# robflynnyh/dynamic-asr-eval

Measured on AMD Instinct MI355X. Metric: audio-sec/s dynamic-eval (fwd+1 adapt step), higher is better.
Workload: dtype f32; 1 GPU; run_dynamic_eval_full: 1 h Earnings-22-shape recording per step (360000 frames, seq_len 16384, overlap 14336, offline, MADGRAD lr 9e-05, 6 freq masks <=34), SCConformerXL 6x768 V+1=4096 seeded weights; windows_per_recording=169, chains_per_gpu=2, lockstep_group=4, hip_graphs=True, pcie_inclusive=False

## Files before the change

dynamic-asr-eval_amd/_lib.py:

```python
import ctypes
import os

_HERE = os.path.dirname(os.path.abspath(__file__))
LIB_PATH = os.environ.get("DYN_LIB_PATH") or os.path.join(_HERE, "libdyneval_hip.so")
_lib = None


class DynError(RuntimeError):
    pass


class GemmDesc(ctypes.Structure):
    _fields_ = [
        ("trans_a", ctypes.c_int32), ("trans_b", ctypes.c_int32),
        ("M", ctypes.c_int64), ("N", ctypes.c_int64), ("K", ctypes.c_int64),
        ("alpha", ctypes.c_float), ("beta", ctypes.c_float),
        ("A", ctypes.c_void_p), ("lda", ctypes.c_int64), ("sa1", ctypes.c_int64), ("sa2", ctypes.c_int64),
        ("B", ctypes.c_void_p), ("ldb", ctypes.c_int64), ("sb1", ctypes.c_int64), ("sb2", ctypes.c_int64),
        ("C", ctypes.c_void_p), ("ldc", ctypes.c_int64), ("sc1", ctypes.c_int64), ("sc2", ctypes.c_int64),
        ("bias", ctypes.c_void_p),
        ("nb1", ctypes.c_int64), ("nb2", ctypes.c_int64),
        ("split_k", ctypes.c_int32),
        ("workspace", ctypes.c_void_p), ("workspace_bytes", ctypes.c_int64),
        ("tile_m", ctypes.c_int32), ("tile_n", ctypes.c_int32), ("tail_slices", ctypes.c_int32), ("reserved_", ctypes.c_int32),
        ("C_in", ctypes.c_void_p),
        ("epilogue", ctypes.c_int32), ("reserved2_", ctypes.c_int32),
        ("aux", ctypes.c_void_p),
        ("a_colsum", ctypes.c_void_p),
        ("a_colsum_beta", ctypes.c_float), ("reserved3_", ctypes.c_float),
        ("counters", ctypes.c_void_p), ("n_counters", ctypes.c_int64),
        ("bias_s1", ctypes.c_int64), ("bias_s2", ctypes.c_int64),
    ]


class DecoderDesc(ctypes.Structure):
    _fields_ = [
        ("d_model", ctypes.c_int32), ("heads", ctypes.c_int32), ("d_ff", ctypes.c_int32), ("vocab", ctypes.c_int32),
        ("layers", ctypes.c_int32), ("n_enc", ctypes.c_int32), ("max_positions", ctypes.c_int32), ("reserved_", ctypes.c_int32),
        ("eps", ctypes.c_float), ("reserved2_", ctypes.c_float),
        ("embed", ctypes.c_void_p), ("pos_table", ctypes.c_void_p), ("norm_out_w", ctypes.c_void_p), ("norm_out_b", ctypes.c_void_p),
        ("head_w", ctypes.c_void_p), ("head_b", ctypes.c_void_p),
        ("layer_ptrs", ctypes.POINTER(ctypes.c_void_p)),
        ("tokens", ctypes.c_void_p), ("logits", ctypes.c_void_p), ("scratch", ctypes.c_void_p), ("scratch_floats", ctypes.c_int64),
    ]


class DecoderBatchDesc(ctypes.Structure):
    _fields_ = [
        ("base", DecoderDesc), ("rows", ctypes.c_int32), ("eos_id", ctypes.c_int32),
        ("token_stride", ctypes.c_int64), ("cache_stride", ctypes.c_int64), ("finished", ctypes.c_void_p),
    ]


DEC_PTRS_PER_LAYER = 18


def load():
    global _lib
    if _lib is not None:
        return _lib
    if not os.path.exists(LIB_PATH):
        raise DynError(
            f"{LIB_PATH} not found: the HIP extension has not been built "
            "(run `python -c 'import __graft_entry__ as g; g.build()'` or `make -C dynamic-asr-eval_amd/csrc`). "
            "There is no CPU fallback for the product path.")
    import torch
    lib = ctypes.CDLL(LIB_PATH)
    for name, (restype, argtypes) in prototypes().items():
        fn = getattr(lib, name)
        fn.restype = restype
        fn.argtypes = argtypes
    _lib = lib
    return lib


def check(rc, what=""):
    if rc != 0:
# ... 44 lines not shown
```

dynamic-asr-eval_amd/csrc/gemm_f32.hip:

```cpp
#include <algorithm>
#include "common.h"
#include <cstdlib>

typedef float f32x16 __attribute__((ext_vector_type(16)));

namespace {

#ifndef DYN_GEMM_BK
#define DYN_GEMM_BK 32
#endif
constexpr int BK = DYN_GEMM_BK;
constexpr int LDK = BK + 4;
constexpr int KV = BK / 4;
constexpr int RP = 256 / KV;
constexpr int NTHREADS = 256;

struct KParams {
    int64_t M, N, K;
    const float* A; int64_t lda, sa1, sa2;
    const float* B; int64_t ldb, sb1, sb2;
    float* C; int64_t ldc, sc1, sc2;
    int64_t cin_delta;
    const float* bias;
    int64_t bs1, bs2;
// ... 488 lines not shown
__global__ void splitk_reduce_kernel(const KParams p) {
    const int64_t mn = p.M * p.N;
    const int64_t total = mn * p.nbatch;
    for (int64_t idx = (int64_t)blockIdx.x * blockDim.x + threadIdx.x; idx < total;
         idx += (int64_t)gridDim.x * blockDim.x) {
        const int64_t zb = idx / mn, rem = idx % mn;
        const int64_t row = rem / p.N, col = rem % p.N;
        float s = 0.f;
        for (int k = 0; k < p.splits; ++k) s += p.ws[((int64_t)k * p.nbatch + zb) * mn + rem];
        const int64_t z1 = zb / p.nb2, z2 = zb % p.nb2;
        float* C = p.C + z1 * p.sc1 + z2 * p.sc2 + row * p.ldc + col;
        float v = epi_value(p.alpha, s, p.beta, C + p.cin_delta, p.bias ? p.bias[z1 * p.bs1 + z2 * p.bs2 + col] : 0.f);
        if (p.epi == 1) { if (p.aux) C[p.aux - p.C] = v; v = silu_f(v); }
        else if (p.epi == 2) v *= silu_grad_f(C[p.aux - p.C]);
        *C = v;
    }
}

__global__ __launch_bounds__(256) void tail_reduce_kernel(const KParams p, int BM, int BN, int64_t tail_items) {
    const int per_tile = BM * BN / 4;
    const int64_t total = tail_items * per_tile;
    for (int64_t idx = (int64_t)blockIdx.x * blockDim.x + threadIdx.x; idx < total; idx += (int64_t)gridDim.x * blockDim.x) {
        const int64_t ti = idx / per_tile;
        const int e4 = (int)(idx % per_tile);
        const int r = (e4 * 4) / BN, c = (e4 * 4) % BN;
        const float4* W = reinterpret_cast<const float4*>(p.tail_ws + (ti * p.tail_f) * (int64_t)(BM * BN)) + e4;
        float4 s4 = W[0];
        for (int k = 1; k < p.tail_f; ++k) {
            const float4 v = W[(int64_t)k * per_tile];
            s4.x += v.x; s4.y += v.y; s4.z += v.z; s4.w += v.w;
        }
        const int64_t item = p.full_items + ti;
        const int tile = (int)(item % p.tiles_per_batch);
        const int zb = (int)(item / p.tiles_per_batch);
        const int64_t row = (int64_t)(p.n_major ? tile % p.tiles_m : tile / p.tiles_n) * BM + r;
        const int64_t col0 = (int64_t)(p.n_major ? tile / p.tiles_m : tile % p.tiles_n) * BN + c;
        if (row >= p.M) continue;
        const int64_t z1 = zb / p.nb2, z2 = zb % p.nb2;
        float* C = p.C + z1 * p.sc1 + z2 * p.sc2 + row * p.ldc;
        const float v[4] = {s4.x, s4.y, s4.z, s4.w};
#pragma unroll
        for (int j = 0; j < 4; ++j) {
            const int64_t col = col0 + j;
            if (col < p.N) {
                float o = epi_value(p.alpha, v[j], p.beta, C + col + p.cin_delta, p.bias ? p.bias[z1 * p.bs1 + z2 * p.bs2 + col] : 0.f);
                if (p.epi == 1) { if (p.aux) C[col + (p.aux - p.C)] = o; o = silu_f(o); }
                else if (p.epi == 2) o *= silu_grad_f(C[col + (p.aux - p.C)]);
                C[col] = o;
            }
        }
    }
}

struct Plan {
    int bm, bn, splits;
    int64_t kchunk;
    int64_t ws_bytes;
    int64_t full_items;
    int64_t tail_items;
    int tail_f;
    int64_t tail_ws_bytes;
};

double tile_eff(int bm, int bn) { return bm == 256 ? 0.84 : (bm == 128 && bn == 128) ? 0.80 : (bm == 64 && bn == 64) ? 0.62 : 0.72; }
int tile_occ(int bm, int bn) { return bm == 256 ? 1 : (bm == 64 && bn == 64) ? 4 : (bm == 128 && bn == 128) ? 2 : 3; }

bool glds_eligible(const dyn_gemm_desc* d) {
    auto al16 = [](const void* q) { return (((uintptr_t)q) & 15) == 0; };
    const bool vec = al16(d->A) && al16(d->B) && (d->lda % 4 == 0) && (d->ldb % 4 == 0) && (d->sa1 % 4 == 0) && (d->sa2 % 4 == 0) &&
                     (d->sb1 % 4 == 0) && (d->sb2 % 4 == 0);
    static const bool allow_glds = [] { const char* e = getenv("DYN_GEMM_GLDS"); return !e || atoi(e) != 0; }();
    const bool ta = d->trans_a != 0, tb = d->trans_b != 0;
    return allow_glds && vec && d->K % BK == 0 && d->K > 0 && (!ta || d->M % 4 == 0) && (tb || d->N % 4 == 0) && (!ta || d->M >= 4) && (tb || d->N >= 4);
}

bool eval_config(const dyn_gemm_desc* d, int bm, int bn, int s, int f_req, Plan* out, double* cost) {
    const int64_t batch = d->nb1 * d->nb2;
    const int64_t ktiles = dyn::cdiv(d->K > 0 ? d->K : 1, BK);
    if (s < 1) s = 1;
    if (s > ktiles) s = (int)ktiles;
    const int64_t tiles = dyn::cdiv(d->M, bm) * dyn::cdiv(d->N, bn);
    const int64_t slots = (int64_t)tile_occ(bm, bn) * 256;
    const int64_t kchunk = dyn::cdiv(ktiles, s) * BK;
    const int s_eff = (int)dyn::cdiv(d->K > 0 ? d->K : 1, kchunk);
    const int64_t items = tiles * batch * s_eff;
    const int64_t rounds = items / slots, rem = items % slots;
    int f = 1;
    if (s_eff == 1 && rem > 0 && f_req != 1) {
        f = f_req > 1 ? f_req : (int)(slots / rem);
        const int64_t maxf = ktiles / 2 > 0 ? ktiles / 2 : 1;
        if (f > maxf) f = (int)maxf;
        if (f > 16) f = 16;
        if (f < 1) f = 1;
    }
    const double round_t = tile_occ(bm, bn) * 2.0 * bm * bn * (double)kchunk / (614e9 * tile_eff(bm, bn));
    double t = rounds * round_t + (rem > 0 ? round_t / f + 1.0e-6 : 0.0);
    if (s_eff > 1) t += 3e-6 + (double)s_eff * d->M * d->N * batch * 4.0 * 2.0 / 3.0e12;
    if (f > 1) t += 2e-6 + (double)f * rem * bm * bn * 4.0 * 2.0 / 3.0e12;
    *cost = t;
    out->bm = bm; out->bn = bn; out->splits = s_eff; out->kchunk = kchunk;
    out->ws_bytes = s_eff > 1 ? (int64_t)s_eff * batch * tiles * bm * bn * (int64_t)sizeof(float) : 0;
    out->tail_f = f;
    out->tail_items = f > 1 ? rem : 0;
    out->full_items = items - out->tail_items;
    out->tail_ws_bytes = f > 1 ? rem * f * (int64_t)bm * bn * (int64_t)sizeof(float) : 0;
    return true;
}

struct Tuned { int ta, tb; int64_t M, N, K, batch; int bm, bn, split, tail; };
#include "gemm_tuned.inc"

Plan make_plan(const dyn_gemm_desc* d) {
    Plan best;
    double cost;
    if (d->tile_m > 0 && d->tile_n > 0) {
        const bool big = d->tile_m >= 256 && d->tile_n >= 128 && glds_eligible(d);
        eval_config(d, big ? 256 : d->tile_m >= 128 ? 128 : 64, d->tile_n >= 128 ? 128 : 64, d->split_k > 0 ? d->split_k : 1,
                    d->tail_slices > 0 ? d->tail_slices : 1, &best, &cost);
        return best;
    }
    const int64_t batch = d->nb1 * d->nb2;
    if (d->split_k == 0) {
        auto less = [](const Tuned& a, const Tuned& b) {
            if (a.ta != b.ta) return a.ta < b.ta;
            if (a.tb != b.tb) return a.tb < b.tb;
            if (a.M != b.M) return a.M < b.M;
            if (a.N != b.N) return a.N < b.N;
            if (a.K != b.K) return a.K < b.K;
            return a.batch < b.batch;
        };
        static const bool sorted = [&] {
            for (int i = 1; i < kNumTuned; ++i)
                if (!less(kTuned[i - 1], kTuned[i])) return false;
            return true;
        }();
        const Tuned want{d->trans_a != 0, d->trans_b != 0, d->M, d->N, d->K, batch, 0, 0, 0, 0};
        const Tuned* hit = nullptr;
        if (sorted) {
            const Tuned* it = std::lower_bound(kTuned, kTuned + kNumTuned, want, less);
            if (it != kTuned + kNumTuned && !less(want, *it)) hit = it;
        } else {
            for (int i = 0; i < kNumTuned && !hit; ++i)
                if (!less(kTuned[i], want) && !less(want, kTuned[i])) hit = &kTuned[i];
        }
        if (hit) {
            eval_config(d, (hit->bm == 256 && !glds_eligible(d)) ? 128 : hit->bm, hit->bn, hit->split, hit->tail, &best, &cost);
            return best;
        }
    }
    const int cand[4][2] = {{128, 128}, {128, 64}, {64, 128}, {64, 64}};
    int split_opts[9] = {1, 2, 3, 4, 6, 8, 12, 16, 24};
    int n_opts = 9;
    if (d->split_k > 0) { split_opts[0] = d->split_k; n_opts = 1; }
    double best_cost = 1e300;
    for (int c = 0; c < 4; ++c) {
        const int bm = cand[c][0], bn = cand[c][1];
        if ((d->M <= 64 && bm == 128) || (d->N <= 64 && bn == 128)) continue;
        for (int so = 0; so < n_opts; ++so) {
            const int s = split_opts[so];
            if (d->split_k == 0 && s > 1 && (d->K / s < 256)) continue;
            Plan pl;
            eval_config(d, bm, bn, s, d->split_k == 0 ? -1 : 1, &pl, &cost);
            if (cost < best_cost) { best_cost = cost; best = pl; }
        }
    }
    return best;
}

template <bool TA, bool TB, int BM, int BN>
void launch_vec(const KParams& kp, bool vec, dim3 grid, hipStream_t st) {
    static const bool allow_glds = [] { const char* e = getenv("DYN_GEMM_GLDS"); return !e || atoi(e) != 0; }();
    const bool glds = allow_glds && vec && kp.K % BK == 0 && kp.K > 0 && (!TA || kp.M % 4 == 0) && (TB || kp.N % 4 == 0) &&
                      (!TA || kp.M >= 4) && (TB || kp.N >= 4);
    if (glds) hipLaunchKernelGGL((gemm_f32_kernel<TA, TB, BM, BN, true, true>), grid, dim3(NTHREADS), 0, st, kp);
    else if (vec) hipLaunchKernelGGL((gemm_f32_kernel<TA, TB, BM, BN, true, false>), grid, dim3(NTHREADS), 0, st, kp);
    else hipLaunchKernelGGL((gemm_f32_kernel<TA, TB, BM, BN, false, false>), grid, dim3(NTHREADS), 0, st, kp);
}

template <bool TA, bool TB>
void launch_tile(const KParams& kp, const Plan& pl, bool vec, dim3 grid, hipStream_t st) {
    if (pl.bm == 256) hipLaunchKernelGGL((gemm_f32_kernel<TA, TB, 256, 128, true, true, 8>), grid, dim3(512), 0, st, kp);
    else if (pl.bm == 128 && pl.bn == 128) launch_vec<TA, TB, 128, 128>(kp, vec, grid, st);
    else if (pl.bm == 128 && pl.bn == 64) launch_vec<TA, TB, 128, 64>(kp, vec, grid, st);
    else if (pl.bm == 64 && pl.bn == 128) launch_vec<TA, TB, 64, 128>(kp, vec, grid, st);
    else launch_vec<TA, TB, 64, 64>(kp, vec, grid, st);
}

}

extern "C" int64_t dyn_gemm_f32_workspace_bytes(const dyn_gemm_desc* d) {
    if (!d || d->M <= 0 || d->N <= 0 || d->nb1 <= 0 || d->nb2 <= 0) return 0;
    const Plan pl = make_plan(d);
    return pl.ws_bytes > pl.tail_ws_bytes ? pl.ws_bytes : pl.tail_ws_bytes;
}

extern "C" int dyn_gemm_f32(const dyn_gemm_desc* d, void* stream) {
    DYN_REQUIRE(d != nullptr, DYN_E_ARG, "dyn_gemm_f32: null descriptor");
    DYN_REQUIRE(d->M >= 0 && d->N >= 0 && d->K >= 0 && d->nb1 >= 1 && d->nb2 >= 1, DYN_E_ARG,
                "dyn_gemm_f32: bad sizes M=%lld N=%lld K=%lld nb=%lldx%lld", (long long)d->M, (long long)d->N,
                (long long)d->K, (long long)d->nb1, (long long)d->nb2);
    if (d->M == 0 || d->N == 0) return DYN_OK;
    DYN_REQUIRE(d->A && d->B && d->C, DYN_E_ARG, "dyn_gemm_f32: null operand");
    DYN_REQUIRE(d->epilogue >= 0 && d->epilogue <= 2 && (d->epilogue != 2 || d->aux), DYN_E_ARG,
                "dyn_gemm_f32: epilogue %d needs 0 <= mode <= 2 (and aux for mode 2)", d->epilogue);
    DYN_REQUIRE(d->a_colsum == nullptr, DYN_E_ARG, "dyn_gemm_f32: a_colsum is a grouped-launch feature (dyn_gemm_f32_grouped)");
    DYN_REQUIRE(d->lda >= (d->trans_a ? d->M : 1) && d->ldb >= (d->trans_b ? d->K : 1) && d->ldc >= d->N,
                DYN_E_ARG, "dyn_gemm_f32: leading dimension smaller than the row length");
    Plan pl = make_plan(d);
    const int64_t need = pl.ws_bytes > pl.tail_ws_bytes ? pl.ws_bytes : pl.tail_ws_bytes;
    if (need > 0 && (d->workspace == nullptr || d->workspace_bytes < need)) {
        DYN_REQUIRE(d->split_k == 0, DYN_E_WORKSPACE, "dyn_gemm_f32: split_k=%d needs %lld workspace bytes, got %lld",
                    d->split_k, (long long)need, (long long)d->workspace_bytes);
        pl.splits = 1;
        pl.kchunk = dyn::cdiv(d->K > 0 ? d->K : 1, BK) * BK;
        pl.ws_bytes = 0; pl.tail_f = 1; pl.tail_items = 0; pl.tail_ws_bytes = 0;
        pl.full_items = dyn::cdiv(d->M, pl.bm) * dyn::cdiv(d->N, pl.bn) * d->nb1 * d->nb2;
    }
    const int64_t batch = d->nb1 * d->nb2;
    KParams kp;
    kp.M = d->M; kp.N = d->N; kp.K = d->K;
    kp.A = d->A; kp.lda = d->lda; kp.sa1 = d->sa1; kp.sa2 = d->sa2;
    kp.B = d->B; kp.ldb = d->ldb; kp.sb1 = d->sb1; kp.sb2 = d->sb2;
    kp.C = d->C; kp.ldc = d->ldc; kp.sc1 = d->sc1; kp.sc2 = d->sc2;
    kp.bias = d->bias; kp.bs1 = d->bias_s1; kp.bs2 = d->bias_s2; kp.alpha = d->alpha; kp.beta = d->beta;
    kp.cin_delta = d->C_in ? (int64_t)(d->C_in - d->C) : 0;
    kp.nb2 = d->nb2; kp.splits = pl.splits; kp.kchunk = pl.kchunk;
    kp.ws = (float*)d->workspace; kp.nbatch = batch;
    const int64_t tiles_m = dyn::cdiv(d->M, pl.bm), tiles_n = dyn::cdiv(d->N, pl.bn);
    kp.tiles_n = (int)tiles_n;
    kp.tiles_m = (int)tiles_m;
    static const bool xcd_map = [] { const char* e = getenv("DYN_GEMM_XCDMAP"); return !e || atoi(e) != 0; }();
    kp.n_major = (xcd_map && d->N > d->M) ? 1 : 0;
    kp.tiles_per_batch = tiles_m * tiles_n;
    kp.full_items = pl.full_items;
    kp.tail_f = pl.tail_f;
    kp.tail_ws = (float*)d->workspace;
    kp.epi = d->epilogue; kp.aux = d->aux;
    const int64_t n_ptiles = pl.splits > 1 ? tiles_m * tiles_n * batch : pl.tail_items;
    kp.counters = (d->counters && n_ptiles > 0 && n_ptiles <= d->n_counters) ? d->counters : nullptr;
    kp.colsum = nullptr; kp.colsum_beta = 0.f; kp.first_item = 0;
    const int64_t nblocks = pl.full_items + pl.tail_items * pl.tail_f;
    DYN_REQUIRE(nblocks < (1ll << 31) && tiles_m * tiles_n < (1ll << 31), DYN_E_ARG, "dyn_gemm_f32: grid too large (%lld workgroups)",
                (long long)nblocks);
    auto al16 = [](const void* q) { return (((uintptr_t)q) & 15) == 0; };
    const bool vec = al16(d->A) && al16(d->B) && (d->lda % 4 == 0) && (d->ldb % 4 == 0) && (d->sa1 % 4 == 0) &&
                     (d->sa2 % 4 == 0) && (d->sb1 % 4 == 0) && (d->sb2 % 4 == 0);
    dim3 grid((unsigned)nblocks);
    hipStream_t st = (hipStream_t)stream;
    if (!d->trans_a && !d->trans_b) launch_tile<false, false>(kp, pl, vec, grid, st);
    else if (!d->trans_a && d->trans_b) launch_tile<false, true>(kp, pl, vec, grid, st);
    else if (d->trans_a && !d->trans_b) launch_tile<true, false>(kp, pl, vec, grid, st);
    else launch_tile<true, true>(kp, pl, vec, grid, st);
    int rc = dyn::check_launch("dyn_gemm_f32");
    if (rc != DYN_OK) return rc;
    if (kp.counters != nullptr) return rc;
    if (pl.splits > 1) {
        const int64_t total = d->M * d->N * batch;
        int64_t nblk = dyn::cdiv(total, 256);
        if (nblk > 2048) nblk = 2048;
        hipLaunchKernelGGL(splitk_reduce_kernel, dim3((unsigned)nblk), dim3(256), 0, st, kp);
        rc = dyn::check_launch("dyn_gemm_f32(splitk_reduce)");
    } else if (pl.tail_items > 0) {
        int64_t nblk = dyn::cdiv(pl.tail_items * pl.bm * pl.bn / 4, 256);
        if (nblk > 4096) nblk = 4096;
        hipLaunchKernelGGL(tail_reduce_kernel, dim3((unsigned)nblk), dim3(256), 0, st, kp, pl.bm, pl.bn, pl.tail_items);
        rc = dyn::check_launch("dyn_gemm_f32(tail_reduce)");
    }
    return rc;
}

extern "C" int64_t dyn_gemm_f32_grouped_workspace_bytes(int32_t n) {
    return (int64_t)(n > 0 ? n : 0) * (int64_t)sizeof(KParams);
}

extern "C" int dyn_gemm_f32_grouped(const dyn_gemm_desc* descs, int32_t n, void* workspace, int64_t workspace_bytes, void* stream) {
    DYN_REQUIRE(descs != nullptr && n >= 0 && n <= kMaxGroups, DYN_E_ARG, "dyn_gemm_f32_grouped: need 0 <= n <= %d descriptors", kMaxGroups);
    if (n == 0) return DYN_OK;
    DYN_REQUIRE(workspace && workspace_bytes >= dyn_gemm_f32_grouped_workspace_bytes(n), DYN_E_WORKSPACE,
                "dyn_gemm_f32_grouped: workspace %lld < %lld bytes", (long long)workspace_bytes,
                (long long)dyn_gemm_f32_grouped_workspace_bytes(n));
    const bool ta = descs[0].trans_a != 0, tb = descs[0].trans_b != 0;
    constexpr int BM = 128, BN = 128;
    auto al16 = [](const void* q) { return (((uintptr_t)q) & 15) == 0; };
    bool glds = true;
    KParams host[kMaxGroups];
    int64_t total = 0;
    int used = 0;
    for (int g = 0; g < n; ++g) {
        const dyn_gemm_desc* d = &descs[g];
        DYN_REQUIRE((d->trans_a != 0) == ta && (d->trans_b != 0) == tb, DYN_E_ARG, "dyn_gemm_f32_grouped: group %d has other transpose flags", g);
        DYN_REQUIRE(d->nb1 == 1 && d->nb2 == 1 && d->split_k == 0 && d->epilogue == 0 && d->bias == nullptr, DYN_E_ARG,
                    "dyn_gemm_f32_grouped: group %d: batches, split-K, bias and activation epilogues are not supported here", g);
        DYN_REQUIRE(d->M >= 0 && d->N >= 0 && d->K >= 0, DYN_E_ARG, "dyn_gemm_f32_grouped: group %d has a negative size", g);
        if (d->M == 0 || d->N == 0) continue;
        DYN_REQUIRE(d->A && d->B && d->C, DYN_E_ARG, "dyn_gemm_f32_grouped: group %d has a null operand", g);
        DYN_REQUIRE(d->lda >= (ta ? d->M : d->K) && d->ldb >= (tb ? d->K : d->N) && d->ldc >= d->N, DYN_E_ARG,
                    "dyn_gemm_f32_grouped: group %d: leading dimension smaller than the row length", g);
        DYN_REQUIRE(al16(d->A) && al16(d->B) && d->lda % 4 == 0 && d->ldb % 4 == 0, DYN_E_ARG,
                    "dyn_gemm_f32_grouped: group %d: operands must be 16-byte aligned with leading dimensions that are multiples of 4", g);
        DYN_REQUIRE(d->a_colsum == nullptr || ta, DYN_E_ARG, "dyn_gemm_f32_grouped: a_colsum needs trans_a (A stored [K][M])");
        glds = glds && d->K % BK == 0 && d->K > 0 && (!ta || (d->M % 4 == 0 && d->M >= 4)) && (tb || (d->N % 4 == 0 && d->N >= 4));
        KParams& kp = host[used++];
// ... 44 lines not shown
```

dynamic-asr-eval_amd/csrc/gemm_tuned.inc:

```
static const Tuned kTuned[] = {
    {0, 0, 32, 64, 32, 24, 64, 64, 1, 8},
    {0, 0, 32, 512, 768, 1, 64, 64, 1, 6},
    {0, 0, 32, 768, 32, 1, 64, 64, 1, 1},
    {0, 0, 32, 3072, 768, 1, 64, 64, 4, 1},
    {0, 0, 32, 6144, 48, 16, 64, 64, 1, 6},
    {0, 0, 64, 64, 64, 24, 64, 64, 1, 6},
    {0, 0, 64, 768, 32, 1, 64, 128, 1, 2},
    {0, 0, 64, 768, 768, 1, 64, 128, 1, 8},
    {0, 0, 64, 3072, 768, 1, 64, 64, 1, 4},
    {0, 0, 96, 64, 96, 12, 64, 64, 1, 8},
    {0, 0, 96, 64, 96, 24, 64, 64, 1, 1},
    {0, 0, 96, 512, 768, 1, 64, 64, 6, 1},
    {0, 0, 96, 768, 768, 1, 64, 64, 1, 6},
    {0, 0, 96, 768, 2304, 1, 64, 64, 1, 8},
    {0, 0, 96, 768, 3072, 1, 64, 64, 1, 8},
    {0, 0, 96, 1024, 512, 1, 64, 64, 1, 4},
    {0, 0, 96, 3072, 768, 1, 64, 64, 2, 1},
    {0, 0, 96, 6144, 48, 16, 64, 64, 1, 2},
    {0, 0, 128, 64, 128, 12, 128, 64, 1, 1},
    {0, 0, 128, 64, 128, 24, 128, 64, 1, 1},
    {0, 0, 128, 512, 768, 1, 64, 64, 1, 8},
    {0, 0, 128, 768, 32, 1, 128, 128, 1, 1},
    {0, 0, 128, 768, 768, 1, 64, 64, 1, 6},
    {0, 0, 128, 768, 2304, 1, 64, 64, 1, 8},
// ... 828 lines not shown
    {0, 1, 1793, 512, 1024, 2, 64, 64, 1, 1},
    {0, 1, 1795, 512, 1536, 2, 64, 64, 1, 1},
    {0, 1, 1800, 512, 1536, 2, 64, 64, 1, 1},
    {0, 1, 1856, 32, 768, 1, 64, 64, 4, 1},
    {0, 1, 1856, 768, 512, 1, 64, 128, 1, 1},
    {0, 1, 1856, 768, 768, 1, 64, 64, 2, 1},
    {0, 1, 1856, 3072, 768, 1, 64, 128, 1, 1},
    {0, 1, 1857, 512, 1024, 2, 64, 64, 1, 1},
    {0, 1, 1920, 32, 768, 1, 64, 64, 4, 1},
    {0, 1, 1920, 768, 512, 1, 64, 64, 1, 1},
    {0, 1, 1920, 768, 768, 1, 64, 64, 1, 2},
    {0, 1, 1920, 2304, 768, 1, 64, 64, 1, 4},
    {0, 1, 1921, 512, 1024, 2, 64, 64, 1, 1},
    {0, 1, 1923, 512, 1536, 2, 64, 64, 1, 1},
    {0, 1, 1984, 32, 768, 1, 64, 64, 1, 4},
    {0, 1, 1984, 768, 512, 1, 64, 64, 1, 1},
    {0, 1, 1984, 768, 768, 1, 64, 64, 1, 2},
    {0, 1, 1984, 768, 3072, 1, 64, 128, 4, 1},
    {0, 1, 1984, 2304, 768, 1, 64, 64, 1, 2},
    {0, 1, 1985, 512, 1024, 2, 64, 64, 1, 1},
    {0, 1, 1992, 768, 768, 1, 64, 64, 1, 1},
    {0, 1, 1992, 768, 768, 2, 64, 64, 1, 1},
    {0, 1, 1992, 768, 768, 3, 64, 64, 1, 2},
    {0, 1, 1992, 768, 768, 4, 64, 128, 1, 8},
    {0, 1, 1992, 768, 768, 6, 64, 64, 1, 1},
    {0, 1, 1992, 768, 768, 8, 64, 128, 1, 4},
    {0, 1, 1992, 768, 2560, 1, 64, 64, 1, 2},
    {0, 1, 1992, 768, 2560, 2, 64, 64, 1, 1},
    {0, 1, 1992, 768, 2560, 3, 64, 64, 1, 4},
    {0, 1, 1992, 768, 2560, 4, 64, 128, 1, 2},
    {0, 1, 1992, 768, 2560, 6, 128, 128, 1, 4},
    {0, 1, 1992, 768, 2560, 8, 128, 128, 1, 2},
    {0, 1, 1992, 768, 3072, 1, 64, 64, 2, 1},
    {0, 1, 1992, 768, 3072, 2, 64, 64, 1, 1},
    {0, 1, 1992, 768, 3072, 3, 64, 64, 1, 2},
    {0, 1, 1992, 768, 3072, 4, 64, 128, 1, 2},
    {0, 1, 1992, 768, 3072, 6, 128, 128, 1, 4},
    {0, 1, 1992, 768, 3072, 8, 128, 128, 1, 3},
    {0, 1, 1992, 768, 4096, 1, 128, 64, 1, 4},
    {0, 1, 1992, 768, 4096, 2, 64, 64, 1, 1},
    {0, 1, 1992, 768, 4096, 3, 64, 64, 1, 2},
    {0, 1, 1992, 768, 4096, 4, 64, 128, 1, 6},
    {0, 1, 1992, 768, 4096, 6, 128, 128, 1, 4},
    {0, 1, 1992, 768, 4096, 8, 128, 128, 1, 2},
    {0, 1, 1992, 1536, 768, 1, 64, 64, 1, 1},
    {0, 1, 1992, 1536, 768, 2, 64, 128, 1, 8},
    {0, 1, 1992, 1536, 768, 3, 128, 128, 1, 4},
    {0, 1, 1992, 1536, 768, 4, 64, 128, 1, 4},
    {0, 1, 1992, 1536, 768, 6, 64, 128, 1, 8},
    {0, 1, 1992, 1536, 768, 8, 256, 128, 1, 4},
    {0, 1, 1992, 1992, 128, 6, 64, 64, 1, 1},
    {0, 1, 1992, 1992, 128, 12, 128, 64, 1, 8},
    {0, 1, 1992, 1992, 128, 18, 128, 64, 1, 6},
    {0, 1, 1992, 1992, 128, 24, 128, 64, 1, 4},
    {0, 1, 1992, 2304, 768, 1, 64, 64, 1, 2},
    {0, 1, 1992, 2304, 768, 2, 128, 128, 1, 3},
    {0, 1, 1992, 2304, 768, 3, 64, 128, 1, 1},
    {0, 1, 1992, 2304, 768, 4, 64, 128, 1, 2},
    {0, 1, 1992, 2304, 768, 6, 128, 128, 1, 1},
    {0, 1, 1992, 2304, 768, 8, 64, 128, 1, 8},
    {0, 1, 1992, 3072, 768, 1, 64, 128, 1, 6},
    {0, 1, 1992, 3072, 768, 2, 64, 128, 1, 6},
    {0, 1, 1992, 3072, 768, 3, 64, 128, 1, 3},
    {0, 1, 1992, 3072, 768, 4, 64, 128, 1, 2},
    {0, 1, 1992, 3072, 768, 6, 64, 128, 1, 8},
    {0, 1, 1992, 3072, 768, 8, 64, 128, 1, 4},
    {0, 1, 1992, 4096, 768, 1, 128, 128, 1, 6},
    {0, 1, 1992, 4096, 768, 2, 128, 128, 1, 1},
    {0, 1, 1992, 4096, 768, 3, 64, 128, 1, 2},
    {0, 1, 1992, 4096, 768, 4, 64, 128, 1, 1},
    {0, 1, 1992, 4096, 768, 6, 64, 128, 1, 2},
    {0, 1, 1992, 4096, 768, 8, 64, 128, 1, 1},
    {0, 1, 2048, 32, 768, 1, 64, 64, 3, 1},
    {0, 1, 2048, 768, 512, 1, 64, 64, 1, 1},
    {0, 1, 2048, 768, 768, 1, 64, 64, 1, 1},
    {0, 1, 2048, 768, 768, 4, 64, 128, 1, 6},
    {0, 1, 2048, 768, 768, 6, 64, 64, 1, 1},
    {0, 1, 2048, 768, 768, 8, 64, 128, 1, 6},
    {0, 1, 2048, 768, 768, 12, 64, 128, 1, 3},
    {0, 1, 2048, 768, 768, 16, 128, 64, 1, 4},
    {0, 1, 2048, 768, 2560, 4, 64, 128, 1, 8},
    {0, 1, 2048, 768, 2560, 6, 128, 128, 1, 4},
    {0, 1, 2048, 768, 2560, 8, 128, 128, 1, 1},
    {0, 1, 2048, 768, 2560, 12, 128, 128, 1, 2},
    {0, 1, 2048, 768, 2560, 16, 256, 128, 1, 2},
    {0, 1, 2048, 768, 3072, 4, 64, 128, 1, 6},
    {0, 1, 2048, 768, 3072, 6, 128, 128, 1, 4},
    {0, 1, 2048, 768, 3072, 8, 128, 128, 1, 2},
    {0, 1, 2048, 768, 3072, 12, 128, 128, 1, 2},
    {0, 1, 2048, 768, 3072, 16, 128, 128, 1, 4},
    {0, 1, 2048, 768, 4096, 4, 128, 64, 1, 3},
    {0, 1, 2048, 768, 4096, 6, 128, 128, 1, 4},
    {0, 1, 2048, 768, 4096, 8, 128, 128, 1, 2},
    {0, 1, 2048, 768, 4096, 12, 128, 128, 1, 2},
    {0, 1, 2048, 768, 4096, 16, 128, 128, 1, 6},
    {0, 1, 2048, 1536, 768, 4, 128, 128, 1, 1},
    {0, 1, 2048, 1536, 768, 6, 64, 128, 1, 2},
    {0, 1, 2048, 1536, 768, 8, 256, 128, 1, 3},
    {0, 1, 2048, 1536, 768, 12, 128, 128, 1, 1},
    {0, 1, 2048, 1536, 768, 16, 128, 128, 1, 6},
    {0, 1, 2048, 2048, 128, 6, 64, 128, 1, 3},
    {0, 1, 2048, 2048, 128, 12, 64, 128, 1, 4},
    {0, 1, 2048, 2048, 128, 18, 64, 128, 1, 8},
    {0, 1, 2048, 2048, 128, 24, 64, 128, 1, 1},
    {0, 1, 2048, 2304, 768, 1, 64, 64, 1, 2},
    {0, 1, 2048, 2304, 768, 4, 64, 128, 1, 8},
    {0, 1, 2048, 2304, 768, 6, 128, 128, 1, 1},
    {0, 1, 2048, 2304, 768, 8, 128, 128, 1, 1},
    {0, 1, 2048, 2304, 768, 12, 128, 128, 1, 1},
    {0, 1, 2048, 2304, 768, 16, 128, 128, 1, 4},
    {0, 1, 2048, 3072, 768, 4, 128, 128, 1, 2},
    {0, 1, 2048, 3072, 768, 6, 128, 128, 1, 1},
    {0, 1, 2048, 3072, 768, 8, 256, 128, 1, 3},
    {0, 1, 2048, 3072, 768, 12, 128, 128, 1, 2},
    {0, 1, 2048, 3072, 768, 16, 256, 128, 1, 4},
    {0, 1, 2048, 4096, 768, 4, 128, 128, 1, 3},
    {0, 1, 2048, 4096, 768, 6, 128, 128, 1, 8},
    {0, 1, 2048, 4096, 768, 8, 128, 128, 1, 2},
    {0, 1, 2048, 4096, 768, 12, 128, 128, 1, 4},
    {0, 1, 2048, 4096, 768, 16, 128, 128, 1, 4},
    {0, 1, 2049, 512, 1024, 2, 64, 64, 1, 4},
    {0, 1, 2051, 512, 1536, 2, 64, 64, 1, 3},
    {0, 1, 2056, 512, 1536, 2, 64, 64, 1, 3},
    {0, 1, 2066, 512, 1536, 2, 64, 64, 4, 1},
    {0, 1, 2086, 512, 1536, 2, 64, 64, 1, 4},
    {0, 1, 2112, 32, 768, 1, 64, 64, 6, 1},
    {0, 1, 2112, 768, 512, 1, 64, 64, 1, 1},
    {0, 1, 2112, 768, 768, 1, 64, 64, 1, 1},
    {0, 1, 2112, 2304, 768, 1, 64, 64, 1, 1},
    {0, 1, 2113, 512, 1024, 2, 64, 64, 1, 1},
    {0, 1, 2176, 32, 768, 1, 64, 64, 3, 1},
    {0, 1, 2176, 768, 512, 1, 64, 64, 1, 1},
    {0, 1, 2176, 768, 768, 1, 64, 64, 1, 1},
    {0, 1, 2176, 2304, 768, 1, 64, 64, 1, 1},
    {0, 1, 2176, 3072, 768, 1, 128, 64, 1, 4},
    {0, 1, 2177, 512, 1024, 2, 64, 64, 1, 4},
    {0, 1, 2179, 512, 1536, 2, 64, 64, 1, 3},
    {0, 1, 2240, 32, 768, 1, 64, 64, 3, 1},
    {0, 1, 2240, 768, 512, 1, 64, 64, 1, 1},
    {0, 1, 2240, 768, 768, 1, 64, 64, 1, 1},
    {0, 1, 2240, 768, 3072, 1, 64, 64, 3, 1},
    {0, 1, 2240, 2304, 768, 1, 64, 64, 1, 1},
    {0, 1, 2240, 3072, 768, 1, 64, 128, 1, 3},
    {0, 1, 2241, 512, 1024, 2, 64, 64, 1, 1},
    {0, 1, 2304, 32, 768, 1, 64, 64, 4, 1},
    {0, 1, 2304, 768, 512, 1, 64, 64, 1, 1},
    {0, 1, 2304, 768, 768, 1, 64, 64, 1, 1},
    {0, 1, 2305, 512, 1024, 2, 64, 64, 1, 1},
    {0, 1, 2307, 512, 1536, 2, 64, 64, 1, 3},
    {0, 1, 2368, 32, 768, 1, 64, 64, 4, 1},
    {0, 1, 2368, 768, 512, 1, 64, 64, 1, 1},
    {0, 1, 2368, 768, 768, 1, 64, 64, 1, 1},
    {0, 1, 2368, 768, 3072, 1, 64, 64, 1, 4},
    {0, 1, 2368, 2304, 768, 1, 64, 128, 1, 1},
    {0, 1, 2368, 3072, 768, 1, 64, 64, 1, 1},
    {0, 1, 2369, 512, 1024, 2, 64, 64, 1, 1},
    {0, 1, 2432, 32, 768, 1, 64, 64, 3, 1},
// ... 673 lines not shown
```

dynamic-asr-eval_amd/ops.py:

```python
import ctypes

import torch

from . import _lib
from ._lib import DynError, GemmDesc, check

_WS = {}
WORKSPACE_BYTES = 1 << 30
F32 = torch.float32
I32 = torch.int32


def _L():
    return _lib.load()


def _stream():
    return torch.cuda.current_stream().cuda_stream


def _chk(t, name, dtype=F32):
    if not isinstance(t, torch.Tensor) or not t.is_cuda:
        raise DynError(f"{name}: expected a CUDA tensor (the HIP path has no CPU fallback)")
    if t.dtype != dtype:
# ... 41 lines not shown
def _is_group(p):
    return isinstance(p, GroupParam)


_WS_OWNER = None


class use_workspace:

    def __init__(self, ws):
        self.ws = ws

    def __enter__(self):
        global _WS_OWNER
        self.prev, _WS_OWNER = _WS_OWNER, self.ws

    def __exit__(self, *exc):
        global _WS_OWNER
        _WS_OWNER = self.prev


def workspace(device=None):
    if _WS_OWNER is not None:
        return _WS_OWNER
    dev = torch.device("cuda", torch.cuda.current_device()) if device is None else torch.device(device)
    idx = dev.index if dev.index is not None else torch.cuda.current_device()
    key = (idx, torch.cuda.current_stream(idx).cuda_stream)
    ws = _WS.get(key)
    if ws is None:
        ws = torch.empty(WORKSPACE_BYTES, dtype=torch.uint8, device=dev)
        _WS[key] = ws
        counters(ws)
    return ws


import os as _os

_COUNTERS = {}
N_COUNTERS = 16384
TICKET_DEFAULT = _os.environ.get("DYN_GEMM_TICKET", "0") == "1"


def counters(ws):
    key = ws.data_ptr()
    c = _COUNTERS.get(key)
    if c is None:
        c = torch.zeros(N_COUNTERS, dtype=torch.int32, device=ws.device)
        _COUNTERS[key] = c
    return c


def gemm(a, b, c, *, trans_a=False, trans_b=False, M, N, K, lda, ldb, ldc, alpha=1.0, beta=0.0, bias=None,
         nb1=1, nb2=1, sa=(0, 0), sb=(0, 0), sc=(0, 0), a_off=0, b_off=0, c_off=0, split_k=0, force=None, c_in=None,
         epilogue=0, aux=None, ticket=None, sbias=(0, 0)):
    _chk(a, "gemm.A"); _chk(b, "gemm.B"); _chk(c, "gemm.C")
    d = GemmDesc()
    if force is not None:
        d.tile_m, d.tile_n, d.tail_slices = force
    d.trans_a, d.trans_b = int(trans_a), int(trans_b)
    d.M, d.N, d.K = M, N, K
    d.alpha, d.beta = alpha, beta
    d.A, d.lda, d.sa1, d.sa2 = a.data_ptr() + 4 * a_off, lda, sa[0], sa[1]
    d.B, d.ldb, d.sb1, d.sb2 = b.data_ptr() + 4 * b_off, ldb, sb[0], sb[1]
    d.C, d.ldc, d.sc1, d.sc2 = c.data_ptr() + 4 * c_off, ldc, sc[0], sc[1]
    d.bias = bias.data_ptr() if bias is not None else None
    d.bias_s1, d.bias_s2 = sbias
    d.C_in = (c_in.data_ptr() + 4 * c_off) if c_in is not None else None
    d.nb1, d.nb2 = nb1, nb2
    d.split_k = split_k
    d.epilogue = int(epilogue)
    d.aux = (aux.data_ptr() + 4 * c_off) if aux is not None else None
    ws = workspace(c.device)
    d.workspace, d.workspace_bytes = ws.data_ptr(), ws.numel()
    if ticket is None:
        ticket = TICKET_DEFAULT
    if ticket:
        cnt = counters(ws)
        d.counters, d.n_counters = cnt.data_ptr(), cnt.numel()
    prof = GEMM_PROFILE
    if prof is not None:
        prof["calls"] += 1
        prof["flops"] += 2.0 * M * N * K * nb1 * nb2
        prof["bytes"] += 4.0 * nb1 * nb2 * (M * K + K * N + M * N * (2 if beta != 0.0 else 1))
        if prof["calls"] % prof["every"] == 0:
            e0, e1 = torch.cuda.Event(enable_timing=True), torch.cuda.Event(enable_timing=True)
            e0.record()
            check(_L().dyn_gemm_f32(ctypes.byref(d), _stream()), "dyn_gemm_f32")
            e1.record()
            prof["samples_excl" if prof.get("exclusive_now") else "samples"].append((2.0 * M * N * K * nb1 * nb2, e0, e1))
            return c
    check(_L().dyn_gemm_f32(ctypes.byref(d), _stream()), "dyn_gemm_f32")
    return c


EPI_SILU, EPI_SILU_GRAD = 1, 2


def wgrad_desc(dy, x, dw, alpha=1.0, beta=1.0, colsum=None, colsum_beta=1.0):
    _cc(dy, "wgrad.dy"); _cc(x, "wgrad.x"); _cc(dw, "wgrad.dw")
    N, K = dw.shape
    M = dy.numel() // N
    d = GemmDesc()
    d.trans_a, d.trans_b = 1, 0
    d.M, d.N, d.K = N, K, M
    d.alpha, d.beta = alpha, beta
    d.A, d.lda = dy.data_ptr(), N
    d.B, d.ldb = x.data_ptr(), K
    d.C, d.ldc = dw.data_ptr(), K
    d.nb1 = d.nb2 = 1
    if colsum is not None:
        _cc(colsum, "wgrad.colsum")
        d.a_colsum, d.a_colsum_beta = colsum.data_ptr(), colsum_beta
    d._keep = (dy, x, dw, colsum)
    return d


MAX_GROUPS = 96


def wgrad_groupable(dy, x, dw):
    N, K = dw.shape
    return N % 4 == 0 and K % 4 == 0 and dy.data_ptr() % 16 == 0 and x.data_ptr() % 16 == 0


def gemm_grouped(descs):
    if len(descs) > MAX_GROUPS:
# ... 1104 lines not shown
```

include/dyneval.h:

```cpp
#ifndef DYNEVAL_H_
#define DYNEVAL_H_
#include <stdint.h>

#ifdef __cplusplus
extern "C" {
#endif

#define DYN_OK 0
#define DYN_E_ARG (-1)
#define DYN_E_LAUNCH (-2)
#define DYN_E_WORKSPACE (-3)
#define DYN_E_UNSUPPORTED (-4)

const char* dyn_last_error(void);
const char* dyn_version(void);
const char* dyn_arch(void);

typedef struct {
    int32_t trans_a, trans_b;
    int64_t M, N, K;
    float alpha, beta;
    const float* A; int64_t lda, sa1, sa2;
    const float* B; int64_t ldb, sb1, sb2;
    float* C;       int64_t ldc, sc1, sc2;
    const float* bias;
    int64_t nb1, nb2;
    int32_t split_k;
    void* workspace; int64_t workspace_bytes;
    int32_t tile_m, tile_n, tail_slices, reserved_;
    const float* C_in;
    int32_t epilogue, reserved2_;
    float* aux;
    float* a_colsum;
    float a_colsum_beta, reserved3_;
    int32_t* counters;
    int64_t n_counters;
    int64_t bias_s1, bias_s2;
} dyn_gemm_desc;

int64_t dyn_gemm_f32_workspace_bytes(const dyn_gemm_desc* d);
int dyn_gemm_f32(const dyn_gemm_desc* d, void* stream);
int64_t dyn_gemm_f32_grouped_workspace_bytes(int32_t n);
int dyn_gemm_f32_grouped(const dyn_gemm_desc* descs, int32_t n, void* workspace, int64_t workspace_bytes, void* stream);

int dyn_gemm_bf16x3_nt(const float* X, const float* W, const float* bias, float* C, int64_t M, int64_t N, int64_t K, int64_t ldx,
                       int64_t ldw, int64_t ldc, void* stream);
int dyn_gemm_bf16x3(int trans_a, int trans_b, const float* A, const float* B, const float* bias, float* C, int64_t M, int64_t N, int64_t K,
                    int64_t lda, int64_t ldb, int64_t ldc, void* stream);
int dyn_bf16x3_split(const float* src, void* planes, int64_t rows, int64_t K, int64_t ld, void* stream);
int dyn_gemm_bf16x3_presplit(const float* X, const void* w_planes, const float* bias, float* C, int64_t M, int64_t N, int64_t K, int64_t ldx,
                             int64_t ldc, void* stream);

int dyn_silu_fwd(const float* x, float* y, int64_t n, void* stream);
int dyn_silu_bwd(const float* x, const float* dy, float* dx, int64_t n, void* stream);
int dyn_glu_fwd(const float* u, float* y, int64_t rows, int64_t C, void* stream);
int dyn_glu_bwd(const float* u, const float* dy, float* du, int64_t rows, int64_t C, void* stream);
int dyn_axpby(const float* x, float* y, float a, float b, int64_t n, void* stream);
int64_t dyn_colsum_workspace_bytes(int64_t rows, int64_t C);
int dyn_colsum(const float* x, float* out, int64_t rows, int64_t C, float beta, void* workspace, int64_t workspace_bytes,
               void* stream);
int dyn_reduce_partials(const float* partial, float* out, int64_t P, int64_t n, float beta, void* stream);
int dyn_reduce_defer_begin(void* arena, int64_t arena_bytes);
int dyn_reduce_defer_flush(void* stream);
int dyn_reduce_defer_abort(void);
int dyn_transpose_ft(const float* x, float* y, int64_t F, int64_t T, int64_t ldx, void* stream);

int64_t dyn_norm_bwd_workspace_bytes(int64_t rows, int64_t C);
int dyn_layernorm_fwd(const float* x, const float* gamma, const float* beta, float* y, float* mean, float* rstd,
                      int64_t rows, int64_t C, float eps, void* stream);
int dyn_layernorm_bwd(const float* x, const float* gamma, const float* mean, const float* rstd, const float* dy, float* dx,
                      float dx_beta, float* dgamma, float* dbeta, float wgrad_beta, int64_t rows, int64_t C,
                      void* workspace, int64_t workspace_bytes, void* stream);
int dyn_layernorm_bwd_res(const float* x, const float* gamma, const float* mean, const float* rstd, const float* dy,
                          const float* dx_in, float* dx, float dx_beta, float* dgamma, float* dbeta, float wgrad_beta,
                          int64_t rows, int64_t C, void* workspace, int64_t workspace_bytes, void* stream);
int dyn_rmsnorm_fwd(const float* x, const float* gamma, float* y, float* rstd, int64_t rows, int64_t C, float eps,
                    void* stream);
int dyn_rmsnorm_bwd(const float* x, const float* gamma, const float* rstd, const float* dy, float* dx, float dx_beta,
                    float* dgamma, float wgrad_beta, int64_t rows, int64_t C, void* workspace, int64_t workspace_bytes,
                    void* stream);
int64_t dyn_norm_bwd_workspace_bytes_g(int64_t rows, int64_t C, int64_t rows_per_sample);
int dyn_layernorm_fwd_g(const float* x, const float* gamma, const float* beta, float* y, float* mean, float* rstd, int64_t rows, int64_t C,
                        float eps, int64_t rows_per_sample, int64_t n_groups, int64_t param_stride, void* stream);
int dyn_layernorm_bwd_g(const float* x, const float* gamma, const float* mean, const float* rstd, const float* dy, const float* dx_in,
                        float* dx, float dx_beta, float* dgamma, float* dbeta, float wgrad_beta, int64_t rows, int64_t C,
                        int64_t rows_per_sample, int64_t n_groups, int64_t param_stride, void* workspace, int64_t workspace_bytes, void* stream);
int dyn_rmsnorm_bwd_g(const float* x, const float* gamma, const float* rstd, const float* dy, float* dx, float dx_beta, float* dgamma,
                      float wgrad_beta, int64_t rows, int64_t C, int64_t rows_per_sample, int64_t n_groups, int64_t param_stride,
                      void* workspace, int64_t workspace_bytes, void* stream);
int dyn_chanaffine_fwd(const float* x, const float* mean, const float* var, const float* weight, const float* bias, float* y,
                       int64_t rows, int64_t C, float eps, void* stream);
int64_t dyn_chanaffine_bwd_workspace_bytes(int64_t rows, int64_t C);
int dyn_chanaffine_bwd(const float* x, const float* mean, const float* var, const float* weight, const float* dy, float* dx,
                       float dx_beta, float* dweight, float* dbias, float wgrad_beta, int64_t rows, int64_t C, float eps,
// ... 256 lines not shown
```

Measured before the change: 797.1 audio-s/s.

## Add stationary-A-panel NT GEMM kernel for small-K attention score products

Adds a specialised NT GEMM kernel for K=64/128 attention-score shapes. It keeps the full A row panel in registers, streams B tiles through a three-stage direct-to-LDS ring, and writes C with DPP quad transposes so stores are float4. The planner picks this form by default when the product is eligible, with no split and no tail, and N is at least 128, or when a tuned entry names it. This is meant to cut repeated A loads and per-tile launch overhead on the score GEMMs. The cost is added register pressure and a new code path whose speed depends on shape.

New measurement: 797.6 audio-s/s, median of 2. No clear change (+0.1%).

```diff
diff --git a/dynamic-asr-eval_amd/_lib.py b/dynamic-asr-eval_amd/_lib.py
--- a/dynamic-asr-eval_amd/_lib.py
+++ b/dynamic-asr-eval_amd/_lib.py
@@ -22,7 +22,7 @@
         ("nb1", ctypes.c_int64), ("nb2", ctypes.c_int64),
         ("split_k", ctypes.c_int32),
         ("workspace", ctypes.c_void_p), ("workspace_bytes", ctypes.c_int64),
-        ("tile_m", ctypes.c_int32), ("tile_n", ctypes.c_int32), ("tail_slices", ctypes.c_int32), ("reserved_", ctypes.c_int32),
+        ("tile_m", ctypes.c_int32), ("tile_n", ctypes.c_int32), ("tail_slices", ctypes.c_int32), ("form", ctypes.c_int32),
         ("C_in", ctypes.c_void_p),
         ("epilogue", ctypes.c_int32), ("reserved2_", ctypes.c_int32),
         ("aux", ctypes.c_void_p),
diff --git a/dynamic-asr-eval_amd/csrc/gemm_f32.hip b/dynamic-asr-eval_amd/csrc/gemm_f32.hip
--- a/dynamic-asr-eval_amd/csrc/gemm_f32.hip
+++ b/dynamic-asr-eval_amd/csrc/gemm_f32.hip
@@ -564,7 +564,142 @@
     }
 }
 
+__device__ __forceinline__ float quad_xor1(float x) { return __builtin_bit_cast(float, __builtin_amdgcn_mov_dpp(__builtin_bit_cast(int, x), 0xB1, 0xF, 0xF, true)); }
+__device__ __forceinline__ float quad_xor2(float x) { return __builtin_bit_cast(float, __builtin_amdgcn_mov_dpp(__builtin_bit_cast(int, x), 0x4E, 0xF, 0xF, true)); }
+__device__ __forceinline__ void quad_transpose(float (&v)[4], int lane) {
+    const bool o1 = (lane & 1) != 0, o2 = (lane & 2) != 0;
+    const float r0 = quad_xor1(o1 ? v[0] : v[1]);
+    const float r1 = quad_xor1(o1 ? v[2] : v[3]);
+    if (o1) { v[0] = r0; v[2] = r1; } else { v[1] = r0; v[3] = r1; }
+    const float r2 = quad_xor2(o2 ? v[0] : v[2]);
+    const float r3 = quad_xor2(o2 ? v[1] : v[3]);
+    if (o2) { v[0] = r2; v[1] = r3; } else { v[2] = r2; v[3] = r3; }
+}
+
+constexpr int kScoresBM = 64, kScoresStages = 3;
+
+template <int N>
+__device__ __forceinline__ void ring_barrier() {
+    asm volatile("s_waitcnt vmcnt(%0) lgkmcnt(0)" ::"n"(N) : "memory");
+    __builtin_amdgcn_s_barrier();
+    asm volatile("" ::: "memory");
+}
+
+template <int BN, int KT>
+__global__ __launch_bounds__(NTHREADS) __attribute__((amdgpu_waves_per_eu(3, 8))) void gemm_scores_nt_kernel(const KParams p) {
+    constexpr int BM = kScoresBM, NS = kScoresStages, WTN = BN / 64, SB = BN * BK;
+    constexpr int NIB = BN / 32;
+    static_assert(BK == 32, "direct-to-LDS staging needs BK = 32");
+    __shared__ __attribute__((aligned(16))) float smem[NS * SB];
+
+    const int64_t bid = blockIdx.x, nwg = p.full_items;
+    const int64_t xcd = bid & 7, xq = nwg >> 3, xr = nwg & 7;
+    const int64_t item = (xcd < xr ? xcd * (xq + 1) : xr * (xq + 1) + (xcd - xr) * xq) + (bid >> 3);
+    const int tm = (int)(item % p.tiles_m);
+    const int64_t zb = item / p.tiles_m;
+    const int64_t z1 = zb / p.nb2, z2 = zb % p.nb2;
+    const float* A = p.A + z1 * p.sa1 + z2 * p.sa2;
+    const float* B = p.B + z1 * p.sb1 + z2 * p.sb2;
+    float* C = p.C + z1 * p.sc1 + z2 * p.sc2;
+    const int64_t m0 = (int64_t)tm * BM;
+    const int tiles_n = p.tiles_n;
+
+    const int lane = threadIdx.x & 63, wave = threadIdx.x >> 6;
+    const int i = lane & 31, h = lane >> 5;
+    const int wm = wave >> 1, wn = wave & 1;
+
+    auto issue_b = [&](int tn, int kt, float* dst) {
+        GldsStager<true, BN> st;
+        st.init(B, p.ldb, (int64_t)tn * BN, p.N, (int64_t)kt * BK, wave, lane);
+        st.issue(dst, wave);
+    };
+    issue_b(0, 0, smem);
+    if (tiles_n * KT > 1) issue_b(1 / KT, 1 % KT, smem + SB);
+
+    float fa[KT][4][4];
+    {
+        int64_t gr = m0 + wm * 32 + i;
+        gr = gr < p.M ? gr : p.M - 1;
+        const float* ap = A + gr * p.lda + 4 * h;
+#pragma unroll
+        for (int kt = 0; kt < KT; ++kt)
+#pragma unroll
+            for (int c = 0; c < 4; ++c) {
+                const float4 v = *reinterpret_cast<const float4*>(ap + 32 * kt + 8 * c);
+                fa[kt][c][0] = v.x; fa[kt][c][1] = v.y; fa[kt][c][2] = v.z; fa[kt][c][3] = v.w;
+            }
+    }
+
+    f32x16 acc[WTN];
+#pragma unroll
+    for (int b = 0; b < WTN; ++b)
+#pragma unroll
+        for (int e = 0; e < 16; ++e) acc[b][e] = 0.f;
+
+    auto store_tile_n = [&](int tn) {
+#pragma unroll
+        for (int b = 0; b < WTN; ++b) {
+            const int64_t col = (int64_t)tn * BN + wn * (BN / 2) + b * 32 + 4 * (i >> 2);
+#pragma unroll
+            for (int g = 0; g < 4; ++g) {
+                float v[4];
+#pragma unroll
+                for (int r = 0; r < 4; ++r) v[r] = epi_value(p.alpha, acc[b][4 * g + r], 0.f, nullptr, 0.f);
+                quad_transpose(v, lane);
+                const int64_t row = m0 + wm * 32 + 8 * g + 4 * h + (i & 3);
+                if (row < p.M && col < p.N) *reinterpret_cast<float4*>(C + row * p.ldc + col) = make_float4(v[0], v[1], v[2], v[3]);
+            }
+#pragma unroll
+            for (int e = 0; e < 16; ++e) acc[b][e] = 0.f;
+        }
+    };
+
+    float fb[2][WTN][4];
+    auto read_b = [&](const float* sb, int c, int slot) {
+#pragma unroll
+        for (int b = 0; b < WTN; ++b) read_frag_glds<true, BN>(sb, wn * (BN / 2) + b * 32, i, h, c, fb[slot][b]);
+    };
+
+    ring_barrier<0>();
+    int buf = 0;
+    read_b(smem, 0, 0);
+    for (int tn = 0; tn < tiles_n; ++tn) {
+#pragma unroll
+        for (int kt = 0; kt < KT; ++kt) {
+            const float* sb = smem + buf * SB;
+            const int b1 = buf + 1 == NS ? 0 : buf + 1, b2 = b1 + 1 == NS ? 0 : b1 + 1;
+            const bool st = kt == 0 && tn > 0;
+            if (st) store_tile_n(tn - 1);
+            const int lkt = (kt + 2) % KT, ltn = tn + (kt + 2) / KT;
+            const bool ld = ltn < tiles_n;
+            if (ld) issue_b(ltn, lkt, smem + b2 * SB);
+#pragma unroll
+            for (int c = 0; c < 3; ++c) {
+                read_b(sb, c + 1, (c + 1) & 1);
+#pragma unroll
+                for (int s = 0; s < 4; ++s)
+#pragma unroll
+                    for (int b = 0; b < WTN; ++b) acc[b] = __builtin_amdgcn_mfma_f32_32x32x2f32(fa[kt][c][s], fb[c & 1][b][s], acc[b], 0, 0, 0);
+                __builtin_amdgcn_sched_group_barrier(0x100, WTN, 0);
+                __builtin_amdgcn_sched_group_barrier(0x008, 4 * WTN, 0);
+            }
+            if (ld) ring_barrier<NIB>();
+            else ring_barrier<0>();
+            if (kt + 1 < KT || tn + 1 < tiles_n) read_b(smem + b1 * SB, 0, 0);
+#pragma unroll
+            for (int s = 0; s < 4; ++s)
+#pragma unroll
+                for (int b = 0; b < WTN; ++b) acc[b] = __builtin_amdgcn_mfma_f32_32x32x2f32(fa[kt][3][s], fb[1][b][s], acc[b], 0, 0, 0);
+            __builtin_amdgcn_sched_group_barrier(0x100, WTN, 0);
+            __builtin_amdgcn_sched_group_barrier(0x008, 4 * WTN, 0);
+            buf = b1;
+        }
+    }
+    store_tile_n(tiles_n - 1);
+}
+
 struct Plan {
+    int form;
     int bm, bn, splits;
     int64_t kchunk;
     int64_t ws_bytes;
@@ -610,6 +745,7 @@
     if (s_eff > 1) t += 3e-6 + (double)s_eff * d->M * d->N * batch * 4.0 * 2.0 / 3.0e12;
     if (f > 1) t += 2e-6 + (double)f * rem * bm * bn * 4.0 * 2.0 / 3.0e12;
     *cost = t;
+    out->form = 0;
     out->bm = bm; out->bn = bn; out->splits = s_eff; out->kchunk = kchunk;
     out->ws_bytes = s_eff > 1 ? (int64_t)s_eff * batch * tiles * bm * bn * (int64_t)sizeof(float) : 0;
     out->tail_f = f;
@@ -619,11 +755,12 @@
     return true;
 }
 
-struct Tuned { int ta, tb; int64_t M, N, K, batch; int bm, bn, split, tail; };
+struct Tuned { int ta, tb; int64_t M, N, K, batch; int bm, bn, split, tail; int form; };
 #include "gemm_tuned.inc"
 
-Plan make_plan(const dyn_gemm_desc* d) {
+Plan make_tile_plan(const dyn_gemm_desc* d, int* tuned_form) {
     Plan best;
+    *tuned_form = -1;
     double cost;
     if (d->tile_m > 0 && d->tile_n > 0) {
         const bool big = d->tile_m >= 256 && d->tile_n >= 128 && glds_eligible(d);
@@ -656,6 +793,7 @@
                 if (!less(kTuned[i], want) && !less(want, kTuned[i])) hit = &kTuned[i];
         }
         if (hit) {
+            *tuned_form = hit->form;
             eval_config(d, (hit->bm == 256 && !glds_eligible(d)) ? 128 : hit->bm, hit->bn, hit->split, hit->tail, &best, &cost);
             return best;
         }
@@ -679,6 +817,31 @@
     return best;
 }
 
+bool scores_eligible(const dyn_gemm_desc* d) {
+    auto al16 = [](const void* q) { return (((uintptr_t)q) & 15) == 0; };
+    return !d->trans_a && d->trans_b && (d->K == 64 || d->K == 128) && d->N % 4 == 0 && d->N >= 4 && d->beta == 0.f && d->bias == nullptr &&
+           d->epilogue == 0 && glds_eligible(d) && al16(d->C) && d->ldc % 4 == 0 && d->sc1 % 4 == 0 && d->sc2 % 4 == 0;
+}
+
+Plan make_plan(const dyn_gemm_desc* d) {
+    int tuned_form;
+    Plan pl = make_tile_plan(d, &tuned_form);
+    if (d->form < 0 || d->split_k != 0 || !scores_eligible(d)) return pl;
+    int bn = 0;
+    if (d->form > 0) {
+        bn = d->form >= 128 ? 128 : 64;
+    } else if (d->tile_m == 0 && pl.splits == 1 && pl.tail_items == 0) {
+        const char* e = getenv("DYN_GEMM_SCORES");
+        if (e && atoi(e) == 0) return pl;
+        bn = tuned_form >= 0 ? tuned_form : (d->N >= 2 * 64 ? 128 : 0);
+    }
+    if (bn == 0) return pl;
+    pl.form = bn; pl.bm = kScoresBM; pl.bn = bn; pl.splits = 1; pl.kchunk = d->K;
+    pl.ws_bytes = 0; pl.tail_f = 1; pl.tail_items = 0; pl.tail_ws_bytes = 0;
+    pl.full_items = dyn::cdiv(d->M, (int64_t)kScoresBM) * d->nb1 * d->nb2;
+    return pl;
+}
+
 template <bool TA, bool TB, int BM, int BN>
 void launch_vec(const KParams& kp, bool vec, dim3 grid, hipStream_t st) {
     static const bool allow_glds = [] { const char* e = getenv("DYN_GEMM_GLDS"); return !e || atoi(e) != 0; }();
@@ -704,6 +867,13 @@
     if (!d || d->M <= 0 || d->N <= 0 || d->nb1 <= 0 || d->nb2 <= 0) return 0;
     const Plan pl = make_plan(d);
     return pl.ws_bytes > pl.tail_ws_bytes ? pl.ws_bytes : pl.tail_ws_bytes;
+}
+
+extern "C" int dyn_gemm_f32_plan(const dyn_gemm_desc* d, int32_t* out5) {
+    DYN_REQUIRE(d != nullptr && out5 != nullptr && d->M > 0 && d->N > 0 && d->nb1 >= 1 && d->nb2 >= 1, DYN_E_ARG, "dyn_gemm_f32_plan: bad arguments");
+    const Plan pl = make_plan(d);
+    out5[0] = pl.form; out5[1] = pl.bm; out5[2] = pl.bn; out5[3] = pl.splits; out5[4] = pl.tail_items > 0 ? pl.tail_f : 1;
+    return DYN_OK;
 }
 
 extern "C" int dyn_gemm_f32(const dyn_gemm_desc* d, void* stream) {
@@ -720,6 +890,7 @@
                 DYN_E_ARG, "dyn_gemm_f32: leading dimension smaller than the row length");
     Plan pl = make_plan(d);
     const int64_t need = pl.ws_bytes > pl.tail_ws_bytes ? pl.ws_bytes : pl.tail_ws_bytes;
+    DYN_REQUIRE(d->form <= 0 || pl.form != 0, DYN_E_ARG, "dyn_gemm_f32: form=%d forced on a product the stationary-panel kernel does not cover", d->form);
     if (need > 0 && (d->workspace == nullptr || d->workspace_bytes < need)) {
         DYN_REQUIRE(d->split_k == 0, DYN_E_WORKSPACE, "dyn_gemm_f32: split_k=%d needs %lld workspace bytes, got %lld",
                     d->split_k, (long long)need, (long long)d->workspace_bytes);
@@ -759,7 +930,13 @@
                      (d->sa2 % 4 == 0) && (d->sb1 % 4 == 0) && (d->sb2 % 4 == 0);
     dim3 grid((unsigned)nblocks);
     hipStream_t st = (hipStream_t)stream;
-    if (!d->trans_a && !d->trans_b) launch_tile<false, false>(kp, pl, vec, grid, st);
+    if (pl.form != 0) {
+#define GO_S(BN_, KT_) hipLaunchKernelGGL((gemm_scores_nt_kernel<BN_, KT_>), grid, dim3(NTHREADS), 0, st, kp)
+        if (pl.form == 128) { if (d->K == 128) GO_S(128, 4); else GO_S(128, 2); }
+        else { if (d->K == 128) GO_S(64, 4); else GO_S(64, 2); }
+#undef GO_S
+    }
+    else if (!d->trans_a && !d->trans_b) launch_tile<false, false>(kp, pl, vec, grid, st);
     else if (!d->trans_a && d->trans_b) launch_tile<false, true>(kp, pl, vec, grid, st);
     else if (d->trans_a && !d->trans_b) launch_tile<true, false>(kp, pl, vec, grid, st);
     else launch_tile<true, true>(kp, pl, vec, grid, st);
diff --git a/dynamic-asr-eval_amd/csrc/gemm_tuned.inc b/dynamic-asr-eval_amd/csrc/gemm_tuned.inc
--- a/dynamic-asr-eval_amd/csrc/gemm_tuned.inc
+++ b/dynamic-asr-eval_amd/csrc/gemm_tuned.inc
@@ -904,7 +904,7 @@
     {0, 1, 1992, 1992, 128, 6, 64, 64, 1, 1},
     {0, 1, 1992, 1992, 128, 12, 128, 64, 1, 8},
     {0, 1, 1992, 1992, 128, 18, 128, 64, 1, 6},
-    {0, 1, 1992, 1992, 128, 24, 128, 64, 1, 4},
+    {0, 1, 1992, 1992, 128, 24, 128, 64, 1, 4, 128},
     {0, 1, 1992, 2304, 768, 1, 64, 64, 1, 2},
     {0, 1, 1992, 2304, 768, 2, 128, 128, 1, 3},
     {0, 1, 1992, 2304, 768, 3, 64, 128, 1, 1},
@@ -954,7 +954,7 @@
     {0, 1, 2048, 2048, 128, 6, 64, 128, 1, 3},
     {0, 1, 2048, 2048, 128, 12, 64, 128, 1, 4},
     {0, 1, 2048, 2048, 128, 18, 64, 128, 1, 8},
-    {0, 1, 2048, 2048, 128, 24, 64, 128, 1, 1},
+    {0, 1, 2048, 2048, 128, 24, 64, 128, 1, 1, 128},
     {0, 1, 2048, 2304, 768, 1, 64, 64, 1, 2},
     {0, 1, 2048, 2304, 768, 4, 64, 128, 1, 8},
     {0, 1, 2048, 2304, 768, 6, 128, 128, 1, 1},
diff --git a/dynamic-asr-eval_amd/ops.py b/dynamic-asr-eval_amd/ops.py
--- a/dynamic-asr-eval_amd/ops.py
+++ b/dynamic-asr-eval_amd/ops.py
@@ -117,7 +117,7 @@
 
 def gemm(a, b, c, *, trans_a=False, trans_b=False, M, N, K, lda, ldb, ldc, alpha=1.0, beta=0.0, bias=None,
          nb1=1, nb2=1, sa=(0, 0), sb=(0, 0), sc=(0, 0), a_off=0, b_off=0, c_off=0, split_k=0, force=None, c_in=None,
-         epilogue=0, aux=None, ticket=None, sbias=(0, 0)):
+         epilogue=0, aux=None, ticket=None, sbias=(0, 0), form=0, plan_only=False):
     _chk(a, "gemm.A"); _chk(b, "gemm.B"); _chk(c, "gemm.C")
     d = GemmDesc()
     if force is not None:
@@ -134,9 +134,14 @@
     d.nb1, d.nb2 = nb1, nb2
     d.split_k = split_k
     d.epilogue = int(epilogue)
+    d.form = int(form)
     d.aux = (aux.data_ptr() + 4 * c_off) if aux is not None else None
     ws = workspace(c.device)
     d.workspace, d.workspace_bytes = ws.data_ptr(), ws.numel()
+    if plan_only:
+        out = (ctypes.c_int32 * 5)()
+        check(_L().dyn_gemm_f32_plan(ctypes.byref(d), out), "dyn_gemm_f32_plan")
+        return dict(zip(("form", "tile_m", "tile_n", "split_k", "tail_slices"), out))
     if ticket is None:
         ticket = TICKET_DEFAULT
     if ticket:
diff --git a/include/dyneval.h b/include/dyneval.h
--- a/include/dyneval.h
+++ b/include/dyneval.h
@@ -27,7 +27,8 @@
     int64_t nb1, nb2;
     int32_t split_k;
     void* workspace; int64_t workspace_bytes;
-    int32_t tile_m, tile_n, tail_slices, reserved_;
+    int32_t tile_m, tile_n, tail_slices;
+    int32_t form;
     const float* C_in;
     int32_t epilogue, reserved2_;
     float* aux;
@@ -40,6 +41,7 @@
 
 int64_t dyn_gemm_f32_workspace_bytes(const dyn_gemm_desc* d);
 int dyn_gemm_f32(const dyn_gemm_desc* d, void* stream);
+int dyn_gemm_f32_plan(const dyn_gemm_desc* d, int32_t* out5);
 int64_t dyn_gemm_f32_grouped_workspace_bytes(int32_t n);
 int dyn_gemm_f32_grouped(const dyn_gemm_desc* descs, int32_t n, void* workspace, int64_t workspace_bytes, void* stream);
 
```
